# danielajisafe/A-NeRF

Hardware: AMD Instinct MI355X
Metric: rays/sec at 512×512×128 samples, 24-joint, 8×256 MLP; 1/2/4/8 GPU (higher is better)
Workload: dtype fp32-accurate split fp16: hidden and view layers after exact power-of-two scaling, x = x0+x1 and W = W0+W1 (remainders within 2^-23 of |x|, |W|), the four fp16 MFMA products x_i W_j (dropped: the remainders' ~2^-22 of |x W|, the bound of bf16x6's dropped terms), fp32 accumulate; the bone-direction a

## Files before the change

### a-nerf_amd/csrc/anerf_kernels.hpp

```cpp
#pragma once

template <int W, int MR, int PREC>
__device__ __forceinline__ void render_item(const ModelDev& M, const RenderArgs& A, const LdsPlan& P,
                                            float* __restrict__ lds, int64_t ray0) {
    constexpr int WH = W / 2;
    const int tid = threadIdx.x, lane = tid & 63, wave = tid >> 6;
    const int R = A.R, S = A.S, I = A.I, T = S + I;
    const int nr = (int)min((int64_t)R, A.n - ray0);

    for (int r = tid; r < nr; r += blockDim.x) {
        const int64_t i = ray0 + r;
        const float* src = A.rb + i * A.stride;
        float* d = lds + P.ray + 16 * r;
        for (int c = 0; c < 6; ++c) d[c] = src[c];
        d[6] = A.cams ? A.cams[i] : -1.0f;
        d[7] = A.near[i];
        d[8] = A.far[i];
        d[9] = norm3(src[3], src[4], src[5]);
        d[10] = __int_as_float(A.ray_pose ? A.ray_pose[i] : 0);
    }
    __syncthreads();
    for (int idx = tid; idx < nr * M.nj * 12; idx += blockDim.x) {
        const int r = idx / (M.nj * 12), e = idx % (M.nj * 12);
        const int j = e / 12, c = e % 12;
        const int pose = __float_as_int(lds[P.ray + 16 * r + 10]);
        lds[P.sk + P.sk_stride * r + e] = (pose >= 0 && pose < A.n_poses) ? A.skts[((int64_t)pose * M.nj + j) * 16 + c]
                                                                           : __int_as_float(0x7fc00000);
    }
    stage_cut(M, lds + P.cut, tid);
    for (int idx = tid; idx < nr * S; idx += blockDim.x) {
        const int r = idx / S, s = idx % S;
        const float t = torch_linspace01(s, S);
        const float nearv = lds[P.ray + 16 * r + 7], farv = lds[P.ray + 16 * r + 8];
        lds[P.zc + P.z_stride * r + s] = lineseg_z(nearv, farv, t, A.lindisp != 0);
    }
    if (A.pass0 == 1) {
        if (T % 4 == 0 && (reinterpret_cast<uintptr_t>(A.zf_ws) & 15) == 0) {
            const f32x4* src = reinterpret_cast<const f32x4*>(A.zf_ws + ray0 * T);
            for (int idx = tid; idx < nr * T / 4; idx += blockDim.x) {
                const int r = (4 * idx) / T, s = (4 * idx) % T;
                *reinterpret_cast<f32x4*>(lds + P.zf + P.z_stride * r + s) = __builtin_nontemporal_load(src + idx);
            }
        } else {
            for (int idx = tid; idx < nr * T; idx += blockDim.x) {
                const int r = idx / T, s = idx % T;
                lds[P.zf + P.z_stride * r + s] = __builtin_nontemporal_load(A.zf_ws + (ray0 + r) * T + s);
            }
        }
    }
    __syncthreads();

    Stamps st;
    STAMP_INIT(st);
    STAMP(st, 0);
    const int n_pass = I > 0 ? 2 : 1;
    for (int pass = A.pass0; pass < min(A.pass1, n_pass); ++pass) {
        const NetDev& net = M.net[pass];
        const int n = pass == 0 ? S : T;
        const int zoff = pass == 0 ? P.zc : P.zf;
        const bool only_new = pass == 1 && M.single_net;
        if (!only_new) {
            stage_bias<W>(M, net, lds + P.bias, tid);
            if (M.mrv == 0) compute_view_factor<WH, 0>(M, net, lds, P, nr, tid, st);
            else compute_view_factor<WH, 4>(M, net, lds, P, nr, tid, st);
        }
        STAMP(st, 1);
        const int nm = only_new ? I : n;
        const int nb = (nm + 31) / 32, nbt = nr * nb;
        auto block_z = [&](int r) {
            return only_new ? lds + P.scr + P.scr_stride * r + 6 * P.z_stride : lds + zoff + P.z_stride * r;
        };
        int* const bcnt = reinterpret_cast<int*>(lds + P.bord);
        int* const bord = bcnt + P.bord_n;
        if constexpr (lockstep_mode<PREC>()) {
            for (int b = wave; b < nbt; b += 4) {
                const int r = b / nb;
                const int c = block_live_count(M, lds + P.ray + 16 * r, lds + P.sk + P.sk_stride * r, lds + P.cut,
                                               block_z(r), nm, (b % nb) * 32, lane);
                if (lane == 0) bcnt[b] = c;
            }
            __syncthreads();
            for (int i = tid; i < nbt; i += blockDim.x) {
                const int ci = bcnt[i];
                int rank = 0;
                for (int j = 0; j < nbt; ++j) {
                    const int cj = bcnt[j];
                    rank += (cj < ci) | ((cj == ci) & (j < i));
                }
                bord[rank] = i;
            }
            __syncthreads();
        }
        for (int it = 0; it < (nbt + 3) / 4; ++it) {
            const bool own = it * 4 + wave < nbt;
            if constexpr (!lockstep_mode<PREC>())
                if (!own) break;
            const int bi = own ? it * 4 + wave : nbt - 1;
            const int b = lockstep_mode<PREC>() ? bord[bi] : bi;
            const int r = b / nb, s0 = (b % nb) * 32;
            const float* zr = block_z(r);
            float* rawr = lds + P.raw + P.raw_stride * r + (only_new ? 4 * S : 0);
            mlp_block<W, MR, PREC>(M, net, lds + P.ray + 16 * r, lds + P.sk + P.sk_stride * r, lds + P.cut,
                             zr, nm, s0, lds + P.g + P.g_stride * r, rawr, lane, own ? A.mfma_count : nullptr,
                             lds + P.bias, (P.uf >= 0 && M.skip + 1 < M.D) ? lds + P.uf + wave * P.uf_stride : nullptr,
                             lds + P.wv + wave * P.wv_stride, st, own);
        }
        STAMP(st, 2 + 2 * pass);
        __syncthreads();
        STAMP(st, 6);
        for (int r0 = 0; r0 < R; r0 += 4) {
            const int r = r0 + __builtin_amdgcn_readfirstlane(wave);
            const bool active = r < nr;
            const int64_t i = ray0 + r;
            const float* ray = lds + P.ray + 16 * min(r, R - 1);
            const float* z = lds + zoff + P.z_stride * min(r, R - 1);
            float* raw = lds + P.raw + P.raw_stride * min(r, R - 1);
            float* scr = lds + P.scr + P.scr_stride * min(r, R - 1);
            if (only_new) {
                const int* src = reinterpret_cast<const int*>(scr + 7 * P.z_stride);
                if (active)
                    for (int k = lane; k < T; k += 64)
                        *reinterpret_cast<f32x4*>(scr + 4 * k) = *reinterpret_cast<const f32x4*>(raw + 4 * src[k]);
                wave_sync();
                if (active)
                    for (int k = lane; k < T; k += 64)
                        *reinterpret_cast<f32x4*>(raw + 4 * k) = *reinterpret_cast<const f32x4*>(scr + 4 * k);
                wave_sync();
            }
            const bool final_pass = pass == n_pass - 1;
            float* o_rgb = final_pass ? A.rgb : A.rgb0;
            float* o_disp = final_pass ? A.disp : A.disp0;
            float* o_acc = final_pass ? A.acc : A.acc0;
            float* o_alpha = final_pass ? A.alpha : A.alpha0;
            float* pal = (active && o_alpha) ? o_alpha + i * n : nullptr;
            if (active) {
                float* dz = pass == 0 ? A.dbg_z0 : A.dbg_z1;
                float* draw = pass == 0 ? A.dbg_raw0 : A.dbg_raw1;
                for (int s = lane; s < n; s += 64) {
                    if (dz) dz[i * n + s] = z[s];
                    if (draw)
                        for (int c = 0; c < 4; ++c) draw[(i * n + s) * 4 + c] = raw[4 * s + c];
                }
            }
            float* res = scr + 7 * P.z_stride;
            composite(M, ray, z, raw, n, scr, P.z_stride, active, lane, pal, res);
            if (active && lane < 5) {
                const float v = res[lane];
                if (lane < 3) {
                    if (o_rgb) o_rgb[3 * i + lane] = v;
                } else if (lane == 3) {
                    if (o_disp) o_disp[i] = v;
                } else if (o_acc) {
                    o_acc[i] = v;
                }
            }
            if (pass == 0 && I > 0) {
                if (active && A.dbg_w0)
                    for (int s = lane; s < S; s += 64) A.dbg_w0[i * S + s] = scr[s];
                importance(z, scr, S, I, lds + P.zf + P.z_stride * min(r, R - 1), scr + P.z_stride, active, lane,
                           nullptr, M.single_net != 0, M.single_net ? reinterpret_cast<int*>(scr + 7 * P.z_stride) : nullptr,
                           M.single_net ? scr + 6 * P.z_stride : nullptr);
            }
        }
        __syncthreads();
        STAMP(st, 3 + 2 * pass);
    }
    if (I > 0 && A.pass1 == 1) {
        if (T % 4 == 0 && (reinterpret_cast<uintptr_t>(A.zf_ws) & 15) == 0) {
            f32x4* dst = reinterpret_cast<f32x4*>(A.zf_ws + ray0 * T);
            for (int idx = tid; idx < nr * T / 4; idx += blockDim.x) {
                const int r = (4 * idx) / T, s = (4 * idx) % T;
                __builtin_nontemporal_store(*reinterpret_cast<const f32x4*>(lds + P.zf + P.z_stride * r + s), dst + idx);
            }
        } else {
            for (int idx = tid; idx < nr * T; idx += blockDim.x) {
                const int r = idx / T, s = idx % T;
                __builtin_nontemporal_store(lds[P.zf + P.z_stride * r + s], A.zf_ws + (ray0 + r) * T + s);
            }
        }
    }
    STAMP_FLUSH(st, A.stamps);
}

template <int W, int MR, int PREC>
__global__ __launch_bounds__(256, 1) void render_kernel(ModelDev M, RenderArgs A, LdsPlan P) {
    extern __shared__ __attribute__((aligned(16))) float lds[];
    const int64_t items = (A.n + A.R - 1) / A.R;
    int* const slot = reinterpret_cast<int*>(lds + P.bord) + 2 * P.bord_n;
    const int g0 = blockIdx.x & 7;
    for (;;) {
        if (threadIdx.x == 0) {
            int64_t item = -1;
            for (int k = 0; k < 8 && item < 0; ++k) {
                const int g = (g0 + k) & 7;
                const int64_t b0 = items * g / 8, b1 = items * (g + 1) / 8;
                if (b1 <= b0) continue;
                const unsigned t = atomicAdd(A.queue + g, 1u);
                if ((int64_t)t < b1 - b0) item = b0 + t;
            }
            slot[0] = (int)item;
        }
        __syncthreads();
        const int item = slot[0];
        if (item < 0) break;
        render_item<W, MR, PREC>(M, A, P, lds, (int64_t)item * A.R);
        __syncthreads();
    }
}

struct DensityArgs {
    const float* pts;
    const float* t;
    const float* kp0;
    int64_t res1;
    int64_t n;
    const float* skts;
    int net;
    float* out;
};

__host__ __device__ inline LdsPlan make_density_plan(int nj, int W, int D, int njh2, bool bone_cut) {
    LdsPlan p;
    std::memset(&p, 0, sizeof(p));
    int o = 0;
    p.sk = o; o += 12 * nj;
    p.cut = o; o += (bone_cut ? 4 : 3) * nj;
    o = (o + 3) & ~3;
    p.bias = o; o += (D + 2) * W;
    p.uf_stride = 64 * 3 * njh2;
    p.uf = o; o += 4 * p.uf_stride;
    p.total = (o + 3) & ~3;
    return p;
}

template <int W, int MR, int PREC>
__global__ __launch_bounds__(256, 1) void density_kernel(ModelDev M, DensityArgs A, LdsPlan P) {
    extern __shared__ __attribute__((aligned(16))) float lds[];
    constexpr int RB = W / 32;
    const int tid = threadIdx.x, lane = tid & 63, wave = tid >> 6, hh = lane >> 5;
    const NetDev& net = M.net[A.net];
// ... 174 lines not shown
        for (int c = 0; c < 3; ++c) {
            const float* wr = net.wrgb + (c * 2 + hh) * RBV * 16;
            float a = 0.0f;
#pragma unroll
            for (int rb = 0; rb < RBV; ++rb)
#pragma unroll
                for (int i = 0; i < 16; ++i) a += wr[rb * 16 + i] * relu_act(av[rb][i]);
            a += __shfl_xor(a, 32);
            if constexpr (PREC >= 3) a *= pow2f(-es);
            rgb[c] = a + net.brgb[c];
        }
        if (own && hh == 0 && s_out < A.n) {
            float* o = A.out + 4 * s_out;
            o[0] = rgb[0];
            o[1] = rgb[1];
            o[2] = rgb[2];
            o[3] = sig;
        }
    }
}

#define ANERF_F16_KERNEL(KW, K, ARGS, WW, MM)                              \
    KW template __global__ void K<WW, MM, 3>(ModelDev, ARGS, LdsPlan);    \
    KW template __global__ void K<WW, MM, 4>(ModelDev, ARGS, LdsPlan);
#ifdef ANERF_AB_FAST
#define ANERF_F16_SHAPES(KW, K, ARGS) ANERF_F16_KERNEL(KW, K, ARGS, 256, 7)
#else
#define ANERF_F16_SHAPES(KW, K, ARGS)                                                                     \
    ANERF_F16_KERNEL(KW, K, ARGS, 256, 7) ANERF_F16_KERNEL(KW, K, ARGS, 128, 7) ANERF_F16_KERNEL(KW, K, ARGS, 64, 7) \
    ANERF_F16_KERNEL(KW, K, ARGS, 256, 10) ANERF_F16_KERNEL(KW, K, ARGS, 128, 10) ANERF_F16_KERNEL(KW, K, ARGS, 64, 10)
#endif
#define ANERF_F16_INSTANCES(KW)                       \
    ANERF_F16_SHAPES(KW, render_kernel, RenderArgs)   \
    ANERF_F16_SHAPES(KW, density_kernel, DensityArgs) \
    ANERF_F16_SHAPES(KW, radiance_kernel, RadianceArgs)
```

### a-nerf_amd/csrc/anerf_kernels_small.hpp

```cpp
#pragma once

__global__ void near_far_given_kernel(const float* __restrict__ rb, int stride, int64_t n, float* __restrict__ near_out,
                                      float* __restrict__ far_out) {
    const int64_t i = (int64_t)blockIdx.x * blockDim.x + threadIdx.x;
    if (i >= n) return;
    near_out[i] = rb[i * stride + 6];
    far_out[i] = rb[i * stride + 7];
}

__global__ void near_far_kernel(const float* __restrict__ rb, int stride, int64_t n, const float* __restrict__ cyls,
                                const int32_t* __restrict__ ray_pose, int n_poses, float* __restrict__ near_out,
                                float* __restrict__ far_out, uint8_t* __restrict__ qnan) {
    const int64_t i = (int64_t)blockIdx.x * blockDim.x + threadIdx.x;
    if (i >= n) return;
    const float* r = rb + i * stride;
    const int pose = ray_pose ? ray_pose[i] : 0;
    if (pose < 0 || pose >= n_poses) {
        near_out[i] = far_out[i] = __int_as_float(0x7fc00000);
        qnan[i] = 1;
        return;
    }
    const float* cy = cyls + 5 * pose;
    const float nearv = r[6], farv = r[7];
    const float rn0 = r[0] + r[3] * nearv, rn1 = r[2] + r[5] * nearv;
// ... 35 lines not shown
    __shared__ int st_a[64], st_b[64];
    __shared__ float st_v[64];
    if (threadIdx.x == 0) n_leaves = np_pairwise_leaves(m, leaf_off, leaf_cnt, NF_LEAVES, st_a, st_b);
    __shared__ float lbuf[NF_LDS];
    float* buf = m <= NF_LDS ? lbuf : scratch + c0;
    for (int v = 0; v < 2; ++v) {
        const float* src = v == 0 ? near_io : far_io;
        int mine = 0;
        for (int64_t i = c0 + threadIdx.x; i < c1; i += blockDim.x) {
            const float x = src[i];
            buf[i - c0] = (x != x) ? 0.0f : x;
            mine += (x == x);
        }
        atomicAdd(&valid[v], mine);
        __syncthreads();
        if (n_leaves >= 0)
            for (int k = threadIdx.x; k < n_leaves; k += blockDim.x) leaf_sum[k] = np_leaf_sum(buf + leaf_off[k], leaf_cnt[k]);
        __syncthreads();
        if (threadIdx.x == 0) {
            const float sum = n_leaves >= 0 ? np_pairwise_combine(leaf_sum, m, st_a, st_b, st_v) : np_pairwise_sum(buf, m);
            means[v] = valid[v] ? (float)((double)sum / (double)valid[v]) : __int_as_float(0x7fc00000);
        }
        __syncthreads();
    }
    for (int64_t i = c0 + threadIdx.x; i < c1; i += blockDim.x) {
        if (qnan[i]) {
            const float* r = rb + i * stride;
            near_io[i] = (means[0] != means[0]) ? r[6] : means[0];
            far_io[i] = (means[1] != means[1]) ? r[7] : means[1];
        }
    }
}

struct PixelSet {
    const int64_t* idx;
    int64_t x0, y0, bw;
    __device__ __forceinline__ int64_t pixel(int64_t t, int W) const {
        return idx ? idx[t] : (y0 + t / bw) * W + x0 + t % bw;
    }
};

__global__ void gen_rays_kernel(const float* __restrict__ c2w, int H, int W, float fx, float fy, float cx, float cy,
                                PixelSet px, int64_t n, float nearv, float farv, float* __restrict__ out) {
    const int64_t t = (int64_t)blockIdx.x * blockDim.x + threadIdx.x;
    if (t >= n) return;
    const int64_t p = px.pixel(t, W);
    const float x = (float)(p % W), y = (float)(p / W);
    const float d0 = (x - cx) / fx;
    const float d1 = -(y - cy) / fy;
    const float d2 = -1.0f;
    float* o = out + t * 11;
    float dd[3];
    for (int r = 0; r < 3; ++r) {
        dd[r] = (d0 * c2w[4 * r + 0] + d1 * c2w[4 * r + 1]) + d2 * c2w[4 * r + 2];
        o[r] = c2w[4 * r + 3];
        o[3 + r] = dd[r];
    }
    o[6] = nearv;
    o[7] = farv;
    const float nn = norm3(dd[0], dd[1], dd[2]);
    o[8] = dd[0] / nn;
    o[9] = dd[1] / nn;
    o[10] = dd[2] / nn;
}

__global__ void compose_fill_kernel(const float* __restrict__ bg, int white, int64_t hw, float* __restrict__ out_rgb,
// ... 74 lines not shown
```

### a-nerf_amd/csrc/anerf_mlp.hpp

```cpp
#pragma once

__device__ __forceinline__ __amdgpu_buffer_rsrc_t make_rsrc(const float* p) {
    return __builtin_amdgcn_make_buffer_rsrc((void*)p, 0, 0x7fffffff, 0x00020000);
}
__device__ __forceinline__ f32x2 bload2(__amdgpu_buffer_rsrc_t rs, int voff, int soff) {
    return __builtin_bit_cast(f32x2, __builtin_amdgcn_raw_buffer_load_b64(rs, voff, soff, 0));
}
__device__ __forceinline__ f32x4 bload4(__amdgpu_buffer_rsrc_t rs, int voff, int soff) {
    return __builtin_bit_cast(f32x4, __builtin_amdgcn_raw_buffer_load_b128(rs, voff, soff, 0));
}

template <int RB>
__device__ __forceinline__ void load_bias(f32x16 (&acc)[RB], const float* __restrict__ bp_lds, int hh) {
#pragma unroll
    for (int rb = 0; rb < RB; ++rb) {
        const f32x4* p = reinterpret_cast<const f32x4*>(bp_lds + (rb * 2 + hh) * 16);
        f32x4 v0 = p[0], v1 = p[1], v2 = p[2], v3 = p[3];
        acc[rb] = f32x16{v0[0], v0[1], v0[2], v0[3], v1[0], v1[1], v1[2], v1[3],
                         v2[0], v2[1], v2[2], v2[3], v3[0], v3[1], v3[2], v3[3]};
    }
}

struct Ring {
    float v[4][16];
// ... 1286 lines not shown
            if constexpr (P == 1)
                mlp_layer_x3<RB, RB>(acc, acc, h, bias + L * W, wl[L], lane, ring, nxt);
            else
                mlp_layer<RB, RB, true, true, false>(acc, acc, h, bias + L * W, wl[L], lane, ring, nxt, nullptr, nosig);
            if (skl && !HANDOFF) ring_preload<2 * RB>(ring, net.wskipu, lane);
        }
        STAMP(st, 11);
        if (skl && enc16) {
            if constexpr (H16) {
                u_part_h<RB, NPH>(acc, M, net.wuh[1], uf, lane, ring, false, pow2f(max(es - net.ewh_u[1], -126)));
                v_part_h<RB, MR, NPH>(acc, M, net.wvh[1], sk, cut, px, py, pz, lane, mask, ring,
                                      pow2f(max(es - net.ewh_v[1], -126)));
            }
            STAMP(st, 12);
        } else if (skl) {
            const float xs = P >= 3 ? pow2f(es) : 1.0f;
            if (ux6) {
                if constexpr (UX6) u_part_x6<RB>(acc, M, net.wskipu6, uf, lane, ring, P == 2, xs);
            } else if (uf)
                u_part_lds<RB>(acc, M, net.wskipu, uf, lane, ring, after, xs);
            else
                u_part<RB, false>(acc, M, net.wskipu, sk, cut, px, py, pz, lane, nullptr, nullptr, nullptr, ring, after,
                                  st, xs);
            if constexpr (VX6)
                v_part_x6<RB, MR>(acc, M, net.wskipv6, sk, cut, px, py, pz, lane, mask, ring, xs);
            else
                v_part<RB, MR>(acc, M, net.wskipv, sk, cut, px, py, pz, lane, mask, st, xs);
            STAMP(st, 12);
        }
    }
    return pre6;
}

template <int W, int MR, int P>
__device__ void mlp_block(const ModelDev& M, const NetDev& net, const float* __restrict__ ray,
                          const float* __restrict__ sk, const float* __restrict__ cut, const float* __restrict__ z,
                          int n, int s0,
                          const float* __restrict__ G, float* __restrict__ raw_out, int lane,
                          unsigned long long* mfma_count, const float* __restrict__ bias, float* __restrict__ uf,
                          float* __restrict__ wvp, Stamps& st, bool store = true) {
    constexpr int RB = W / 32;
    constexpr int RBV = (W / 2) / 32;
    const int sl = lane & 31, hh = lane >> 5;
    int s = s0 + sl;
    if (s >= n) s = n - 1;
    const float zs = z[s];
    const float px = ray[0] + ray[3] * zs;
    const float py = ray[1] + ray[4] * zs;
    const float pz = ray[2] + ray[5] * zs;

    f32x16 acc[RB], h[RB];
    JointMask mask;
    Ring ring;
    int es = 0;
    const bool pre = mlp_trunk<W, MR, true, P>(M, net, sk, cut, px, py, pz, lane, bias, uf, wvp, acc, h, ring, mask,
                                               P >= 3 ? net.wviewh : (P == 2 ? net.wview6 : net.wview), st, es);
    float sig = 0.0f;
    f32x16 av[RBV];
    if constexpr (P >= 3) {
        const int es_h = es;
        mlp_layer_h3<RBV, RB, false, true, P == 4 ? 4 : 3>(av, acc, h, nullptr, net.wviewh, lane, ring, pre, nullptr,
                                           bias + (M.D + 1) * W, sig, es, net.ew_view, M.h3_top);
        sig *= pow2f(-es_h);
    } else if constexpr (P == 2)
        mlp_layer_x6<RBV, RB, false, true>(av, acc, h, nullptr, net.wview6, lane, ring, pre, nullptr,
                                           bias + (M.D + 1) * W, sig);
    else
// ... 17 lines not shown
            for (int i = 0; i < 16; ++i) a += wr[rb * 16 + i] * relu_act(av[rb][i]);
        if constexpr (P >= 3) a = sum_halves(a);
        else a += __shfl_xor(a, 32);
        if constexpr (P >= 3) a *= pow2f(-es);
        rgb[c] = a + net.brgb[c];
    }
    STAMP(st, 13);
    if (mfma_count && lane == 0) {
        const int act = __builtin_popcountll(mask.m0) + __builtin_popcountll(mask.m1);
        const bool ux6 = (P >= 2) && (RB % 4 == 0) && uf != nullptr;
        constexpr bool vx6 = (P >= 2) && (RB % 4 == 0);
        const int npe = (P >= 3 && ux6 && M.enc16) ? (P == 4 ? 4 : 3) : 6;
        const int xk = (ux6 ? 0 : 3 * M.njh2) + (vx6 ? 0 : act * VPart<MR>::KB);
        long long k = (long long)xk * RB + (long long)vsteps * RBV;
        const int nx = (M.skip + 1 < M.D) ? 2 : 1;
        if (ux6) atomicAdd(mfma_count + 1, (unsigned long long)(nx * ((3 * M.njh2 + 7) / 8) * RB * npe));
        if (vx6) atomicAdd(mfma_count + 1, (unsigned long long)(nx * act * VPartX6<MR, 1>::KS * RB * npe));
        constexpr int NPR = P == 2 ? 6 : (P == 4 ? 4 : 3);
        if (P >= 2)
            atomicAdd(mfma_count + 1, (unsigned long long)(RBV * RB * 2 * NPR));
        else
            k += (long long)(W / 2) * RBV;
        if (M.skip + 1 < M.D) k += (long long)xk * RB;
        const long long hid = (long long)(M.D - 1) * RB * RB;
        if (P != 0) {
            atomicAdd(mfma_count + 1, (unsigned long long)(hid * 2 * NPR));
        } else {
            k += hid * 16;
        }
        atomicAdd(mfma_count, (unsigned long long)k);
    }
    if (store && hh == 0 && s0 + sl < n) {
        float* o = raw_out + 4 * (s0 + sl);
        o[0] = rgb[0];
        o[1] = rgb[1];
        o[2] = rgb[2];
        o[3] = sig;
    }
}
```

### a-nerf_amd/csrc/anerf_render.hip

```cpp
#include <hip/hip_runtime.h>

#include <algorithm>
#include <cmath>
#include <cstdio>
#include <cstdlib>
#include <cstring>
#include <string>
#include <type_traits>
#include <vector>

#include "../../include/anerf.h"
#include "anerf_device.hpp"

using namespace anerf;

#include "anerf_types.hpp"
#include "anerf_mlp.hpp"
#include "anerf_stages.hpp"
#include "anerf_kernels.hpp"
ANERF_F16_INSTANCES(extern)
#include "anerf_kernels_small.hpp"
#include "anerf_train.hpp"
#include "anerf_trainfwd.hpp"
#include "anerf_pose.hpp"
// ... 185 lines not shown
    if (embed->cutoff_dist || embed->cutoff_dist_v || cb) {
        const size_t nb = sizeof(float) * (size_t)m->desc.n_joints;
        int prev = 0;
        HIP_TRY(hipGetDevice(&prev));
        HIP_TRY(hipSetDevice(m->device));
        hipError_t e = hipDeviceSynchronize();
        if (e == hipSuccess && embed->cutoff_dist)
            e = hipMemcpy(const_cast<float*>(m->md.cutoff), embed->cutoff_dist,
                          m->md.kp_query ? 3 * sizeof(float) : nb, hipMemcpyHostToDevice);
        if (e == hipSuccess && embed->cutoff_dist_v)
            e = hipMemcpy(const_cast<float*>(m->md.cutoff_v), embed->cutoff_dist_v, nb, hipMemcpyHostToDevice);
        if (e == hipSuccess && cb)
            e = hipMemcpy(const_cast<float*>(m->md.cutoff_b), embed->cutoff_dist_b, nb, hipMemcpyHostToDevice);
        (void)hipSetDevice(prev);
        if (e != hipSuccess) return fail(ANERF_EHIP, std::string("anerf_model_set_embed: ") + hipGetErrorString(e));
    }
    m->md.tau = embed->tau;
    m->md.tau_v = embed->tau_v;
    if (btab) m->md.tau_b = embed->tau_b;
    if (embed->cutoff_dist && !m->md.kp_query) m->cut_host.assign(embed->cutoff_dist, embed->cutoff_dist + m->desc.n_joints);
    if (!m->md.staged) enc16_units(m);
    return ANERF_OK;
}

static size_t ws_near_far_bytes(int64_t n) {
    auto al = [](size_t x) { return (x + 255) & ~(size_t)255; };
    return 3 * al(sizeof(float) * (size_t)n) + al((size_t)n);
}

static size_t ws_zf_bytes(int64_t n, int32_t n_samples, int32_t n_importance) {
    return n_importance > 0 ? (((size_t)n * (size_t)(n_samples + n_importance) * 4 + 255) & ~(size_t)255) : 0;
}

size_t anerf_workspace_size(const anerf_model* m, int64_t n_rays, int32_t n_samples, int32_t n_importance) {
    (void)m;
    const int64_t n = n_rays > 0 ? n_rays : 1;
    return ws_near_far_bytes(n) + ws_zf_bytes(n, n_samples, n_importance) + 256;
}

static int launch_near_far(const float* rb, int stride, int64_t n, const float* cyls, const int32_t* ray_pose,
                           int n_poses, int chunk, char* ws, float** near_o, float** far_o, hipStream_t st) {
    auto al = [](size_t x) { return (x + 255) & ~(size_t)255; };
    float* nearp = reinterpret_cast<float*>(ws);
    float* farp = reinterpret_cast<float*>(ws + al(sizeof(float) * n));
    float* scratch = reinterpret_cast<float*>(ws + 2 * al(sizeof(float) * n));
    uint8_t* qnan = reinterpret_cast<uint8_t*>(ws + 3 * al(sizeof(float) * n));
    const int bs = 256;
    hipLaunchKernelGGL(near_far_kernel, dim3((unsigned)((n + bs - 1) / bs)), dim3(bs), 0, st, rb, stride, n, cyls,
                       ray_pose, n_poses, nearp, farp, qnan);
    const int64_t nchunks = (n + chunk - 1) / chunk;
    hipLaunchKernelGGL(nan_fill_kernel, dim3((unsigned)nchunks), dim3(256), 0, st, rb, stride, n, chunk, nearp, farp,
                       qnan, scratch);
    HIP_TRY(hipGetLastError());
    *near_o = nearp;
    *far_o = farp;
    return ANERF_OK;
}

int anerf_near_far(const float* ray_batch, int32_t ray_stride, int64_t n_rays, const float* cyls, int32_t n_poses,
                   const int32_t* ray_pose, int32_t chunk, float* near_out, float* far_out, void* workspace,
                   size_t workspace_bytes, void* stream) {
    if (n_rays <= 0) return ANERF_OK;
    if (!ray_batch || !cyls || !near_out || !far_out || ray_stride < 8 || chunk <= 0 || n_poses < 1)
        return fail(ANERF_EINVAL, "anerf_near_far: bad arguments");
    if (!workspace || workspace_bytes < ws_near_far_bytes(n_rays)) return fail(ANERF_EWORKSPACE, "workspace too small");
    hipStream_t st = reinterpret_cast<hipStream_t>(stream);
    float *np_, *fp_;
    int rc = launch_near_far(ray_batch, ray_stride, n_rays, cyls, ray_pose, n_poses, chunk,
                             (char*)workspace, &np_, &fp_, st);
    if (rc) return rc;
// ... 25 lines not shown
        return fail(ANERF_EINVAL, "n_importance > 0 needs a fine network (or a single_net model)");
    if (n_importance > 0 && n_samples < 3) return fail(ANERF_EINVAL, "importance sampling needs n_samples >= 3");
    if (m->desc.framecode_ch > 0 && !cams) return fail(ANERF_EINVAL, "model uses framecodes: cams required");
    if (chunk <= 0) return fail(ANERF_EINVAL, "chunk must be > 0");
    if (!workspace || workspace_bytes < anerf_workspace_size(m, n_rays, n_samples, n_importance))
        return fail(ANERF_EWORKSPACE, "workspace too small");
    int dev = -1;
    HIP_TRY(hipGetDevice(&dev));
    if (dev != m->device) return fail(ANERF_EINVAL, "current device differs from the model's device");
    hipStream_t st = reinterpret_cast<hipStream_t>(stream);

    float *nearp, *farp;
    if (flags & ANERF_FLAG_NEAR_FAR) {
        auto al = [](size_t x) { return (x + 255) & ~(size_t)255; };
        nearp = reinterpret_cast<float*>(workspace);
        farp = reinterpret_cast<float*>((char*)workspace + al(sizeof(float) * n_rays));
        hipLaunchKernelGGL(near_far_given_kernel, dim3((unsigned)((n_rays + 255) / 256)), dim3(256), 0, st, ray_batch,
                           ray_stride, n_rays, nearp, farp);
        HIP_TRY(hipGetLastError());
    } else {
        int rc = launch_near_far(ray_batch, ray_stride, n_rays, cyls, ray_pose, n_poses, chunk, (char*)workspace,
                                 &nearp, &farp, st);
        if (rc) return rc;
    }
    if (debug && debug->near) HIP_TRY(hipMemcpyAsync(debug->near, nearp, 4 * n_rays, hipMemcpyDeviceToDevice, st));
    if (debug && debug->far) HIP_TRY(hipMemcpyAsync(debug->far, farp, 4 * n_rays, hipMemcpyDeviceToDevice, st));

    const int S = n_samples, I = n_importance, T = S + I;
    const int nbc = (S + 31) / 32;
    int R = std::max(4, 8 / nbc);
    R = std::min(R, 8);
    const int W = m->desc.net_width;
    const int nj = m->desc.n_joints, mrv = layout_multires_views(m->desc.multires_views), D = m->desc.net_depth;
    LdsPlan P = make_plan(R, nj, W, S, T, mrv, m->ngh, D, m->njh2, true, m->md.bone_cut != 0);
    if (P.total * 4 > 160 * 1024) P = make_plan(R, nj, W, S, T, mrv, m->ngh, D, m->njh2, false, m->md.bone_cut != 0);
    while (R > 1 && P.total * 4 > 160 * 1024) {
        R /= 2;
        P = make_plan(R, nj, W, S, T, mrv, m->ngh, D, m->njh2, false, m->md.bone_cut != 0);
    }
    if (P.total * 4 > 160 * 1024) return fail(ANERF_EINVAL, "configuration exceeds the 160 KiB LDS budget");

    RenderArgs a;
    std::memset(&a, 0, sizeof(a));
    a.rb = ray_batch;
    a.n = n_rays;
    a.stride = ray_stride;
    a.S = S;
    a.I = I;
    a.R = R;
    a.skts = skts;
    a.n_poses = n_poses;
    a.ray_pose = ray_pose;
    a.cams = cams;
    a.near = nearp;
    a.far = farp;
    a.rgb = rgb;
    a.disp = disp;
    a.acc = acc;
    a.rgb0 = rgb0;
    a.disp0 = disp0;
    a.acc0 = acc0;
    a.alpha = alpha;
    a.alpha0 = alpha0;
    a.lindisp = (flags & ANERF_FLAG_LINDISP) ? 1 : 0;
    if (debug) {
        a.dbg_z0 = debug->z_coarse;
        a.dbg_raw0 = debug->raw_coarse;
        a.dbg_w0 = debug->weights0;
        a.dbg_z1 = debug->z_fine;
        a.dbg_raw1 = debug->raw_fine;
        a.mfma_count = debug->mfma_count;
    }
#ifdef ANERF_STAMPS
    a.stamps = g_stamps;
#endif
    const int pstep = (I > 0 && !m->desc.single_net) ? 1 : 2;
    a.zf_ws = I > 0 ? reinterpret_cast<float*>((char*)workspace + ws_near_far_bytes(n_rays)) : nullptr;
    unsigned grid = (unsigned)((n_rays + R - 1) / R);
    unsigned* queues = reinterpret_cast<unsigned*>((char*)workspace + ws_near_far_bytes(n_rays) +
                                                   ws_zf_bytes(n_rays, S, I));
    int ncu = 256;
    (void)hipDeviceGetAttribute(&ncu, hipDeviceAttributeMultiprocessorCount, dev);
    HIP_TRY(hipMemsetAsync(queues, 0, 2 * 8 * sizeof(unsigned), st));
    const size_t lds_bytes = (size_t)P.total * 4;
    const int mr = layout_multires(m->desc.multires);
#define ANERF_LAUNCH(WW, MM)                                                                         \
    do {                                                                                            \
        auto kfn = precision == ANERF_PREC_BF16X3 ? render_kernel<WW, MM, 1>                       \
                 : precision == ANERF_PREC_BF16X6 ? render_kernel<WW, MM, 2>                       \
                 : precision == ANERF_PREC_FP16X3 ? render_kernel<WW, MM, 3>                       \
                 : precision == ANERF_PREC_FP16X4 ? render_kernel<WW, MM, 4> : render_kernel<WW, MM, 0>; \
        HIP_TRY(hipFuncSetAttribute((const void*)kfn, hipFuncAttributeMaxDynamicSharedMemorySize,  \
                                    (int)lds_bytes));                                               \
        int nb = 1;                                                                                 \
        if (hipOccupancyMaxActiveBlocksPerMultiprocessor(&nb, kfn, 256, lds_bytes) != hipSuccess || nb < 1) \
            nb = 1;                                                                                 \
        const unsigned g = std::min<unsigned>(grid, (unsigned)(ncu * nb));                          \
        for (int p0 = 0; p0 < 2; p0 += pstep) {                                                     \
            a.pass0 = p0;                                                                           \
            a.pass1 = p0 + pstep;                                                                   \
            a.queue = queues + 8 * p0;                                                              \
            hipLaunchKernelGGL(kfn, dim3(g), dim3(256), lds_bytes, st, m->md, a, P);               \
        }                                                                                           \
    } while (0)
    if (W == 256 && mr == 7) ANERF_LAUNCH(256, 7);
#ifndef ANERF_AB_FAST
    else if (W == 128 && mr == 7) ANERF_LAUNCH(128, 7);
    else if (W == 64 && mr == 7) ANERF_LAUNCH(64, 7);
    else if (W == 256 && mr == 10) ANERF_LAUNCH(256, 10);
    else if (W == 128 && mr == 10) ANERF_LAUNCH(128, 10);
    else if (W == 64 && mr == 10) ANERF_LAUNCH(64, 10);
#endif
    else return fail(ANERF_EINVAL, "no kernel instance for this width / multires");
#undef ANERF_LAUNCH
    HIP_TRY(hipGetLastError());
    return ANERF_OK;
}

int anerf_gen_rays(const float* c2w, int32_t H, int32_t W, float focal_x, float focal_y, float center_x,
                   float center_y, int32_t has_center, const int64_t* idx, int64_t n, float nearv, float farv,
                   float* ray_batch_out, void* stream) {
    if (n == 0) return ANERF_OK;
    if (!c2w || !idx || !ray_batch_out || H <= 0 || W <= 0 || n < 0) return fail(ANERF_EINVAL, "anerf_gen_rays: bad arguments");
    const float cx = has_center ? center_x : (float)(W * 0.5);
    const float cy = has_center ? center_y : (float)(H * 0.5);
    hipStream_t st = reinterpret_cast<hipStream_t>(stream);
    hipLaunchKernelGGL(gen_rays_kernel, dim3((unsigned)((n + 255) / 256)), dim3(256), 0, st, c2w, H, W, focal_x,
                       focal_y, cx, cy, PixelSet{idx, 0, 0, 1}, n, nearv, farv, ray_batch_out);
    HIP_TRY(hipGetLastError());
    return ANERF_OK;
}

int anerf_gen_rays_box(const float* c2w, int32_t H, int32_t W, float focal_x, float focal_y, float center_x,
                       float center_y, int32_t has_center, int32_t x0, int32_t y0, int32_t x1, int32_t y1, float nearv,
                       float farv, float* ray_batch_out, void* stream) {
    if (!c2w || !ray_batch_out || H <= 0 || W <= 0 || x0 < 0 || y0 < 0 || x1 > W || y1 > H)
        return fail(ANERF_EINVAL, "anerf_gen_rays_box: bad arguments");
    if (x1 <= x0 || y1 <= y0) return ANERF_OK;
    const int64_t n = (int64_t)(x1 - x0) * (y1 - y0);
    const float cx = has_center ? center_x : (float)(W * 0.5);
    const float cy = has_center ? center_y : (float)(H * 0.5);
    hipStream_t st = reinterpret_cast<hipStream_t>(stream);
    hipLaunchKernelGGL(gen_rays_kernel, dim3((unsigned)((n + 255) / 256)), dim3(256), 0, st, c2w, H, W, focal_x,
                       focal_y, cx, cy, PixelSet{nullptr, x0, y0, x1 - x0}, n, nearv, farv, ray_batch_out);
    HIP_TRY(hipGetLastError());
    return ANERF_OK;
}
// ... 674 lines not shown
```

### a-nerf_amd/csrc/anerf_types.hpp

```cpp
#pragma once


struct Stamps {
#ifdef ANERF_STAMPS
    unsigned long long last, acc[24];
#endif
};
#ifdef ANERF_STAMPS
#define STAMP_INIT(st)                                      \
    do {                                                    \
        (st).last = __builtin_amdgcn_s_memtime();           \
        for (int i_ = 0; i_ < 24; ++i_) (st).acc[i_] = 0;   \
    } while (0)
#define STAMP(st, i)                                                      \
    do {                                                                  \
        __builtin_amdgcn_sched_barrier(0);                                \
        const unsigned long long now_ = __builtin_amdgcn_s_memtime();     \
        (st).acc[i] += now_ - (st).last;                                  \
        (st).last = now_;                                                 \
        __builtin_amdgcn_sched_barrier(0);                                \
    } while (0)
#define STAMP_FLUSH(st, ptr)                                              \
    do {                                                                  \
        if ((threadIdx.x & 63) == 0 && (ptr))                             \
// ... 50 lines not shown
    int sparse;
    int single_net;
    int cut_to, shift_in;
    int h3_top;
    int bone_cut;
    int view_raw;
    int mrb, kp_relpos, view_angle, bone_win, staged;
    int kp_query;
    int view_win;
    int enc16;
    float shift, B, tau, tau_v, tau_b;
    const float* cutoff;
    const float* cutoff_v;
    const float* cutoff_b;
    NetDev net[2];
};

struct RenderArgs {
    const float* rb;
    int64_t n;
    int stride, S, I, R;
    int n_poses;
    const float* skts;
    const int32_t* ray_pose;
    const float* cams;
    const float* near;
    const float* far;
    float *rgb, *disp, *acc, *rgb0, *disp0, *acc0, *alpha, *alpha0;
    float *dbg_z0, *dbg_raw0, *dbg_w0, *dbg_z1, *dbg_raw1;
    unsigned long long* mfma_count;
    unsigned long long* stamps;
    int pass0, pass1;
    float* zf_ws;
    int lindisp;
    unsigned* queue;
};

struct LdsPlan {
    int ray, sk, zc, zf, raw, g, scr, bias, cut, uf, wv;
    int bord, bord_n;
    int total;
    int sk_stride, z_stride, raw_stride, g_stride, scr_stride, uf_stride, wv_stride;
};

__host__ __device__ inline int pad32(int x) { return (x + 31) & ~31; }

__device__ __forceinline__ void kp_inputs(int cut_to, int shift_in, float dist, float c, float& u, float& uf) {
    u = cut_to ? c - dist : dist;
    uf = shift_in ? u * (2.0f / c) - 1.0f : u;
}

__host__ __device__ inline LdsPlan make_plan(int R, int nj, int W, int S, int T, int mrv, int ngh, int D, int njh2,
                                             bool with_uf, bool bone_cut) {
    LdsPlan p;
    const int wh = W / 2;
    const int nk = 1 + 2 * mrv;
    p.sk_stride = nj * 12;
    p.z_stride = pad32(T > S ? T : S);
    p.raw_stride = p.z_stride * 4;
    p.g_stride = 2 * ngh * wh;
    int scr_a = 8 * p.z_stride;
    int scr_b = ((3 * nk + 3) & ~3) * nj + 256;
    p.scr_stride = (scr_a > scr_b ? scr_a : scr_b);
    int o = 0;
    p.ray = o; o += 16 * R;
    p.sk = o; o += p.sk_stride * R;
    p.zc = o; o += p.z_stride * R;
    p.zf = o; o += p.z_stride * R;
    p.raw = o; o += p.raw_stride * R;
    p.g = o; o += p.g_stride * R;
    p.scr = o; o += p.scr_stride * R;
    o = (o + 3) & ~3;
    p.bias = o; o += (D + 2) * W;
    p.cut = o; o += (bone_cut ? 4 : 3) * nj;
    o = (o + 3) & ~3;
    p.uf_stride = 64 * 3 * njh2;
    p.uf = with_uf ? o : -1;
    if (with_uf) o += 4 * p.uf_stride;
    p.wv_stride = 64 * (njh2 + 1);
    p.wv = o; o += 4 * p.wv_stride;
    p.bord_n = (R * (((T > S ? T : S) + 31) / 32) + 3) & ~3;
    p.bord = o; o += 2 * p.bord_n + 4;
    p.total = (o + 3) & ~3;
    return p;
}
```

Before: 1.231 million.

## Split compositing and importance sampling into separate per-ray stage kernels

When the coarse and fine networks are separate, the render kernel now only evaluates the MLP and writes raw outputs to a global workspace with nontemporal vector stores. New 64-thread per-ray kernels then do compositing, importance sampling and the output maps. Dropping raw, fine-z and large scratch buffers shrinks the MLP kernel's LDS plan, and the serial per-ray compositing work leaves the MFMA-heavy kernel. The cost is extra global memory traffic for the raw buffer, extra kernel launches and a larger workspace. The old fused path stays for single-net models.

```diff
diff --git a/a-nerf_amd/csrc/anerf_kernels.hpp b/a-nerf_amd/csrc/anerf_kernels.hpp
--- a/a-nerf_amd/csrc/anerf_kernels.hpp
+++ b/a-nerf_amd/csrc/anerf_kernels.hpp
@@ -1,6 +1,6 @@
 #pragma once
 
-template <int W, int MR, int PREC>
+template <int W, int MR, int PREC, bool FUSED>
 __device__ __forceinline__ void render_item(const ModelDev& M, const RenderArgs& A, const LdsPlan& P,
                                             float* __restrict__ lds, int64_t ray0) {
     constexpr int WH = W / 2;
@@ -28,13 +28,14 @@
                                                                            : __int_as_float(0x7fc00000);
     }
     stage_cut(M, lds + P.cut, tid);
-    for (int idx = tid; idx < nr * S; idx += blockDim.x) {
-        const int r = idx / S, s = idx % S;
-        const float t = torch_linspace01(s, S);
-        const float nearv = lds[P.ray + 16 * r + 7], farv = lds[P.ray + 16 * r + 8];
-        lds[P.zc + P.z_stride * r + s] = lineseg_z(nearv, farv, t, A.lindisp != 0);
-    }
-    if (A.pass0 == 1) {
+    if (FUSED || A.pass0 == 0)
+        for (int idx = tid; idx < nr * S; idx += blockDim.x) {
+            const int r = idx / S, s = idx % S;
+            const float t = torch_linspace01(s, S);
+            const float nearv = lds[P.ray + 16 * r + 7], farv = lds[P.ray + 16 * r + 8];
+            lds[P.zc + P.z_stride * r + s] = lineseg_z(nearv, farv, t, A.lindisp != 0);
+        }
+    if (!FUSED && A.pass0 == 1) {
         if (T % 4 == 0 && (reinterpret_cast<uintptr_t>(A.zf_ws) & 15) == 0) {
             const f32x4* src = reinterpret_cast<const f32x4*>(A.zf_ws + ray0 * T);
             for (int idx = tid; idx < nr * T / 4; idx += blockDim.x) {
@@ -58,7 +59,7 @@
         const NetDev& net = M.net[pass];
         const int n = pass == 0 ? S : T;
         const int zoff = pass == 0 ? P.zc : P.zf;
-        const bool only_new = pass == 1 && M.single_net;
+        const bool only_new = FUSED && pass == 1 && M.single_net;
         if (!only_new) {
             stage_bias<W>(M, net, lds + P.bias, tid);
             if (M.mrv == 0) compute_view_factor<WH, 0>(M, net, lds, P, nr, tid, st);
@@ -99,13 +100,15 @@
             const int b = lockstep_mode<PREC>() ? bord[bi] : bi;
             const int r = b / nb, s0 = (b % nb) * 32;
             const float* zr = block_z(r);
-            float* rawr = lds + P.raw + P.raw_stride * r + (only_new ? 4 * S : 0);
-            mlp_block<W, MR, PREC>(M, net, lds + P.ray + 16 * r, lds + P.sk + P.sk_stride * r, lds + P.cut,
+            float* rawr = FUSED ? lds + P.raw + P.raw_stride * r + (only_new ? 4 * S : 0)
+                                : A.raw_ws + (ray0 + r) * n * 4;
+            mlp_block<W, MR, PREC, !FUSED>(M, net, lds + P.ray + 16 * r, lds + P.sk + P.sk_stride * r, lds + P.cut,
                              zr, nm, s0, lds + P.g + P.g_stride * r, rawr, lane, own ? A.mfma_count : nullptr,
                              lds + P.bias, (P.uf >= 0 && M.skip + 1 < M.D) ? lds + P.uf + wave * P.uf_stride : nullptr,
                              lds + P.wv + wave * P.wv_stride, st, own);
         }
         STAMP(st, 2 + 2 * pass);
+        if constexpr (!FUSED) break;
         __syncthreads();
         STAMP(st, 6);
         for (int r0 = 0; r0 < R; r0 += 4) {
@@ -165,25 +168,11 @@
         __syncthreads();
         STAMP(st, 3 + 2 * pass);
     }
-    if (I > 0 && A.pass1 == 1) {
-        if (T % 4 == 0 && (reinterpret_cast<uintptr_t>(A.zf_ws) & 15) == 0) {
-            f32x4* dst = reinterpret_cast<f32x4*>(A.zf_ws + ray0 * T);
-            for (int idx = tid; idx < nr * T / 4; idx += blockDim.x) {
-                const int r = (4 * idx) / T, s = (4 * idx) % T;
-                __builtin_nontemporal_store(*reinterpret_cast<const f32x4*>(lds + P.zf + P.z_stride * r + s), dst + idx);
-            }
-        } else {
-            for (int idx = tid; idx < nr * T; idx += blockDim.x) {
-                const int r = idx / T, s = idx % T;
-                __builtin_nontemporal_store(lds[P.zf + P.z_stride * r + s], A.zf_ws + (ray0 + r) * T + s);
-            }
-        }
-    }
     STAMP_FLUSH(st, A.stamps);
 }
 
-template <int W, int MR, int PREC>
-__global__ __launch_bounds__(256, 1) void render_kernel(ModelDev M, RenderArgs A, LdsPlan P) {
+template <int W, int MR, int PREC, bool FUSED>
+__device__ __forceinline__ void render_items(const ModelDev& M, const RenderArgs& A, const LdsPlan& P) {
     extern __shared__ __attribute__((aligned(16))) float lds[];
     const int64_t items = (A.n + A.R - 1) / A.R;
     int* const slot = reinterpret_cast<int*>(lds + P.bord) + 2 * P.bord_n;
@@ -203,9 +192,19 @@
         __syncthreads();
         const int item = slot[0];
         if (item < 0) break;
-        render_item<W, MR, PREC>(M, A, P, lds, (int64_t)item * A.R);
+        render_item<W, MR, PREC, FUSED>(M, A, P, lds, (int64_t)item * A.R);
         __syncthreads();
     }
+}
+
+template <int W, int MR, int PREC>
+__global__ __launch_bounds__(256, 1) void render_kernel(ModelDev M, RenderArgs A, LdsPlan P) {
+    render_items<W, MR, PREC, false>(M, A, P);
+}
+
+template <int W, int MR, int PREC>
+__global__ __launch_bounds__(256, 1) void render_fused_kernel(ModelDev M, RenderArgs A, LdsPlan P) {
+    render_items<W, MR, PREC, true>(M, A, P);
 }
 
 struct DensityArgs {
@@ -446,5 +445,6 @@
 #endif
 #define ANERF_F16_INSTANCES(KW)                       \
     ANERF_F16_SHAPES(KW, render_kernel, RenderArgs)   \
+    ANERF_F16_SHAPES(KW, render_fused_kernel, RenderArgs) \
     ANERF_F16_SHAPES(KW, density_kernel, DensityArgs) \
     ANERF_F16_SHAPES(KW, radiance_kernel, RadianceArgs)
diff --git a/a-nerf_amd/csrc/anerf_kernels_small.hpp b/a-nerf_amd/csrc/anerf_kernels_small.hpp
--- a/a-nerf_amd/csrc/anerf_kernels_small.hpp
+++ b/a-nerf_amd/csrc/anerf_kernels_small.hpp
@@ -91,6 +91,81 @@
     }
 }
 
+__host__ __device__ inline int render_stage_lds_floats(int S, int I, bool coarse) {
+    return 16 + ((coarse && I > 0) ? 10 : 9) * pad32(S + I);
+}
+
+__device__ __forceinline__ void render_stage_maps(const float* res, int lane, int64_t i, float* __restrict__ o_rgb,
+                                                  float* __restrict__ o_disp, float* __restrict__ o_acc) {
+    if (lane < 5) {
+        const float v = res[lane];
+        if (lane < 3) {
+            if (o_rgb) o_rgb[3 * i + lane] = v;
+        } else if (lane == 3) {
+            if (o_disp) o_disp[i] = v;
+        } else if (o_acc) {
+            o_acc[i] = v;
+        }
+    }
+}
+
+__global__ __launch_bounds__(64) void render_coarse_stage_kernel(ModelDev M, RenderArgs A) {
+    extern __shared__ __attribute__((aligned(16))) float lds[];
+    const int64_t i = blockIdx.x;
+    const int lane = threadIdx.x, S = A.S, I = A.I, T = S + I;
+    const int zs = pad32(T);
+    float* ray = lds;
+    float* z = lds + 16;
+    float* zf = z + zs;
+    float* scr = I > 0 ? zf + zs : zf;
+    const float* src = A.rb + i * A.stride;
+    if (lane == 0) ray[9] = norm3(src[3], src[4], src[5]);
+    const float nearv = A.near[i], farv = A.far[i];
+    for (int s = lane; s < S; s += 64) z[s] = lineseg_z(nearv, farv, torch_linspace01(s, S), A.lindisp != 0);
+    wave_sync();
+    const float* raw = A.raw_ws + i * S * 4;
+    const bool final_pass = I == 0;
+    float* o_alpha = final_pass ? A.alpha : A.alpha0;
+    for (int s = lane; s < S; s += 64) {
+        if (A.dbg_z0) A.dbg_z0[i * S + s] = z[s];
+        if (A.dbg_raw0)
+            for (int c = 0; c < 4; ++c) A.dbg_raw0[(i * S + s) * 4 + c] = raw[4 * s + c];
+    }
+    float* res = scr + 7 * zs;
+    composite(M, ray, z, raw, S, scr, zs, true, lane, o_alpha ? o_alpha + i * S : nullptr, res);
+    render_stage_maps(res, lane, i, final_pass ? A.rgb : A.rgb0, final_pass ? A.disp : A.disp0,
+                      final_pass ? A.acc : A.acc0);
+    if (I > 0) {
+        if (A.dbg_w0)
+            for (int s = lane; s < S; s += 64) A.dbg_w0[i * S + s] = scr[s];
+        [[clang::always_inline]] importance(z, scr, S, I, zf, scr + zs, true, lane);
+        for (int s = lane; s < T; s += 64) A.zf_ws[i * T + s] = zf[s];
+    }
+}
+
+__global__ __launch_bounds__(64) void render_fine_stage_kernel(ModelDev M, RenderArgs A) {
+    extern __shared__ __attribute__((aligned(16))) float lds[];
+    const int64_t i = blockIdx.x;
+    const int lane = threadIdx.x, T = A.S + A.I;
+    const int zs = pad32(T);
+    float* ray = lds;
+    float* z = lds + 16;
+    float* scr = z + zs;
+    const float* src = A.rb + i * A.stride;
+    if (lane == 0) ray[9] = norm3(src[3], src[4], src[5]);
+    for (int s = lane; s < T; s += 64) z[s] = A.zf_ws[i * T + s];
+    wave_sync();
+    const float* raw = A.raw_ws + i * T * 4;
+    for (int s = lane; s < T; s += 64) {
+        if (A.dbg_z1) A.dbg_z1[i * T + s] = z[s];
+        if (A.dbg_raw1)
+            for (int c = 0; c < 4; ++c) A.dbg_raw1[(i * T + s) * 4 + c] = raw[4 * s + c];
+    }
+    float* res = scr + 7 * zs;
+    composite(M, ray, z, raw, T, scr, zs, true, lane, A.alpha ? A.alpha + i * T : nullptr, res);
+    render_stage_maps(res, lane, i, A.rgb, A.disp, A.acc);
+}
+
 struct PixelSet {
     const int64_t* idx;
     int64_t x0, y0, bw;
diff --git a/a-nerf_amd/csrc/anerf_mlp.hpp b/a-nerf_amd/csrc/anerf_mlp.hpp
--- a/a-nerf_amd/csrc/anerf_mlp.hpp
+++ b/a-nerf_amd/csrc/anerf_mlp.hpp
@@ -1342,7 +1342,7 @@
     return pre6;
 }
 
-template <int W, int MR, int P>
+template <int W, int MR, int P, bool GRAW = false>
 __device__ void mlp_block(const ModelDev& M, const NetDev& net, const float* __restrict__ ray,
                           const float* __restrict__ sk, const float* __restrict__ cut, const float* __restrict__ z,
                           int n, int s0,
@@ -1426,9 +1426,14 @@
     }
     if (store && hh == 0 && s0 + sl < n) {
         float* o = raw_out + 4 * (s0 + sl);
-        o[0] = rgb[0];
-        o[1] = rgb[1];
-        o[2] = rgb[2];
-        o[3] = sig;
-    }
-}
+        if constexpr (GRAW) {
+            const f32x4 v = {rgb[0], rgb[1], rgb[2], sig};
+            __builtin_nontemporal_store(v, reinterpret_cast<f32x4*>(o));
+        } else {
+            o[0] = rgb[0];
+            o[1] = rgb[1];
+            o[2] = rgb[2];
+            o[3] = sig;
+        }
+    }
+}
diff --git a/a-nerf_amd/csrc/anerf_render.hip b/a-nerf_amd/csrc/anerf_render.hip
--- a/a-nerf_amd/csrc/anerf_render.hip
+++ b/a-nerf_amd/csrc/anerf_render.hip
@@ -241,10 +241,15 @@
     return n_importance > 0 ? (((size_t)n * (size_t)(n_samples + n_importance) * 4 + 255) & ~(size_t)255) : 0;
 }
 
+static size_t ws_raw_bytes(const anerf_model* m, int64_t n, int32_t n_samples, int32_t n_importance) {
+    if (m && m->desc.single_net) return 0;
+    return ((size_t)n * (size_t)(n_samples + n_importance) * 16 + 255) & ~(size_t)255;
+}
+
 size_t anerf_workspace_size(const anerf_model* m, int64_t n_rays, int32_t n_samples, int32_t n_importance) {
-    (void)m;
     const int64_t n = n_rays > 0 ? n_rays : 1;
-    return ws_near_far_bytes(n) + ws_zf_bytes(n, n_samples, n_importance) + 256;
+    return ws_near_far_bytes(n) + ws_zf_bytes(n, n_samples, n_importance) + ws_raw_bytes(m, n, n_samples, n_importance) +
+           256;
 }
 
 static int launch_near_far(const float* rb, int stride, int64_t n, const float* cyls, const int32_t* ray_pose,
@@ -336,13 +341,26 @@
     R = std::min(R, 8);
     const int W = m->desc.net_width;
     const int nj = m->desc.n_joints, mrv = layout_multires_views(m->desc.multires_views), D = m->desc.net_depth;
-    LdsPlan P = make_plan(R, nj, W, S, T, mrv, m->ngh, D, m->njh2, true, m->md.bone_cut != 0);
-    if (P.total * 4 > 160 * 1024) P = make_plan(R, nj, W, S, T, mrv, m->ngh, D, m->njh2, false, m->md.bone_cut != 0);
+    const bool fused = m->desc.single_net != 0;
+    LdsPlan P = make_plan(R, nj, W, S, T, mrv, m->ngh, D, m->njh2, true, m->md.bone_cut != 0, fused);
+    if (P.total * 4 > 160 * 1024)
+        P = make_plan(R, nj, W, S, T, mrv, m->ngh, D, m->njh2, false, m->md.bone_cut != 0, fused);
     while (R > 1 && P.total * 4 > 160 * 1024) {
         R /= 2;
-        P = make_plan(R, nj, W, S, T, mrv, m->ngh, D, m->njh2, false, m->md.bone_cut != 0);
+        P = make_plan(R, nj, W, S, T, mrv, m->ngh, D, m->njh2, false, m->md.bone_cut != 0, fused);
     }
     if (P.total * 4 > 160 * 1024) return fail(ANERF_EINVAL, "configuration exceeds the 160 KiB LDS budget");
+    const size_t stage_lds[2] = {sizeof(float) * render_stage_lds_floats(S, I, true),
+                                 sizeof(float) * render_stage_lds_floats(S, I, false)};
+    if (!fused) {
+        if (stage_lds[0] > 160 * 1024) return fail(ANERF_EINVAL, "configuration exceeds the 160 KiB LDS budget");
+        if (stage_lds[0] > 64 * 1024)
+            HIP_TRY(hipFuncSetAttribute((const void*)render_coarse_stage_kernel,
+                                        hipFuncAttributeMaxDynamicSharedMemorySize, (int)stage_lds[0]));
+        if (I > 0 && stage_lds[1] > 64 * 1024)
+            HIP_TRY(hipFuncSetAttribute((const void*)render_fine_stage_kernel,
+                                        hipFuncAttributeMaxDynamicSharedMemorySize, (int)stage_lds[1]));
+    }
 
     RenderArgs a;
     std::memset(&a, 0, sizeof(a));
@@ -378,33 +396,46 @@
 #ifdef ANERF_STAMPS
     a.stamps = g_stamps;
 #endif
-    const int pstep = (I > 0 && !m->desc.single_net) ? 1 : 2;
+    const int pstep = fused ? 2 : 1;
+    const int n_launch = fused ? 1 : (I > 0 ? 2 : 1);
     a.zf_ws = I > 0 ? reinterpret_cast<float*>((char*)workspace + ws_near_far_bytes(n_rays)) : nullptr;
+    a.raw_ws = fused ? nullptr
+                     : reinterpret_cast<float*>((char*)workspace + ws_near_far_bytes(n_rays) + ws_zf_bytes(n_rays, S, I));
     unsigned grid = (unsigned)((n_rays + R - 1) / R);
     unsigned* queues = reinterpret_cast<unsigned*>((char*)workspace + ws_near_far_bytes(n_rays) +
-                                                   ws_zf_bytes(n_rays, S, I));
+                                                   ws_zf_bytes(n_rays, S, I) + ws_raw_bytes(m, n_rays, S, I));
     int ncu = 256;
     (void)hipDeviceGetAttribute(&ncu, hipDeviceAttributeMultiprocessorCount, dev);
     HIP_TRY(hipMemsetAsync(queues, 0, 2 * 8 * sizeof(unsigned), st));
     const size_t lds_bytes = (size_t)P.total * 4;
     const int mr = layout_multires(m->desc.multires);
+#define ANERF_PICK(K, WW, MM)                                                  \
+    (precision == ANERF_PREC_BF16X3 ? K<WW, MM, 1>                             \
+     : precision == ANERF_PREC_BF16X6 ? K<WW, MM, 2>                           \
+     : precision == ANERF_PREC_FP16X3 ? K<WW, MM, 3>                           \
+     : precision == ANERF_PREC_FP16X4 ? K<WW, MM, 4> : K<WW, MM, 0>)
 #define ANERF_LAUNCH(WW, MM)                                                                         \
     do {                                                                                            \
-        auto kfn = precision == ANERF_PREC_BF16X3 ? render_kernel<WW, MM, 1>                       \
-                 : precision == ANERF_PREC_BF16X6 ? render_kernel<WW, MM, 2>                       \
-                 : precision == ANERF_PREC_FP16X3 ? render_kernel<WW, MM, 3>                       \
-                 : precision == ANERF_PREC_FP16X4 ? render_kernel<WW, MM, 4> : render_kernel<WW, MM, 0>; \
+        auto kfn = fused ? ANERF_PICK(render_fused_kernel, WW, MM) : ANERF_PICK(render_kernel, WW, MM); \
         HIP_TRY(hipFuncSetAttribute((const void*)kfn, hipFuncAttributeMaxDynamicSharedMemorySize,  \
                                     (int)lds_bytes));                                               \
         int nb = 1;                                                                                 \
         if (hipOccupancyMaxActiveBlocksPerMultiprocessor(&nb, kfn, 256, lds_bytes) != hipSuccess || nb < 1) \
             nb = 1;                                                                                 \
         const unsigned g = std::min<unsigned>(grid, (unsigned)(ncu * nb));                          \
-        for (int p0 = 0; p0 < 2; p0 += pstep) {                                                     \
+        for (int p0 = 0; p0 < n_launch; ++p0) {                                                     \
             a.pass0 = p0;                                                                           \
             a.pass1 = p0 + pstep;                                                                   \
             a.queue = queues + 8 * p0;                                                              \
             hipLaunchKernelGGL(kfn, dim3(g), dim3(256), lds_bytes, st, m->md, a, P);               \
+            if (!fused) {                                                                           \
+                if (p0 == 0)                                                                        \
+                    hipLaunchKernelGGL(render_coarse_stage_kernel, dim3((unsigned)n_rays), dim3(64), stage_lds[0], st, \
+                                       m->md, a);                                                   \
+                else                                                                                \
+                    hipLaunchKernelGGL(render_fine_stage_kernel, dim3((unsigned)n_rays), dim3(64), stage_lds[1], st, \
+                                       m->md, a);                                                   \
+            }                                                                                       \
         }                                                                                           \
     } while (0)
     if (W == 256 && mr == 7) ANERF_LAUNCH(256, 7);
@@ -417,6 +448,7 @@
 #endif
     else return fail(ANERF_EINVAL, "no kernel instance for this width / multires");
 #undef ANERF_LAUNCH
+#undef ANERF_PICK
     HIP_TRY(hipGetLastError());
     return ANERF_OK;
 }
diff --git a/a-nerf_amd/csrc/anerf_types.hpp b/a-nerf_amd/csrc/anerf_types.hpp
--- a/a-nerf_amd/csrc/anerf_types.hpp
+++ b/a-nerf_amd/csrc/anerf_types.hpp
@@ -106,6 +106,7 @@
     unsigned long long* stamps;
     int pass0, pass1;
     float* zf_ws;
+    float* raw_ws;
     int lindisp;
     unsigned* queue;
 };
@@ -125,22 +126,23 @@
 }
 
 __host__ __device__ inline LdsPlan make_plan(int R, int nj, int W, int S, int T, int mrv, int ngh, int D, int njh2,
-                                             bool with_uf, bool bone_cut) {
+                                             bool with_uf, bool bone_cut, bool fused) {
     LdsPlan p;
     const int wh = W / 2;
     const int nk = 1 + 2 * mrv;
     p.sk_stride = nj * 12;
     p.z_stride = pad32(T > S ? T : S);
-    p.raw_stride = p.z_stride * 4;
+    p.raw_stride = fused ? p.z_stride * 4 : 0;
     p.g_stride = 2 * ngh * wh;
-    int scr_a = 8 * p.z_stride;
+    int scr_a = fused ? 8 * p.z_stride : 0;
     int scr_b = ((3 * nk + 3) & ~3) * nj + 256;
     p.scr_stride = (scr_a > scr_b ? scr_a : scr_b);
     int o = 0;
     p.ray = o; o += 16 * R;
     p.sk = o; o += p.sk_stride * R;
     p.zc = o; o += p.z_stride * R;
-    p.zf = o; o += p.z_stride * R;
+    p.zf = fused ? o : p.zc;
+    if (fused) o += p.z_stride * R;
     p.raw = o; o += p.raw_stride * R;
     p.g = o; o += p.g_stride * R;
     p.scr = o; o += p.scr_stride * R;
```

Result: faster. 1.254 million (median of 6 runs) (+1.8%).
